# HKUST-Aerial-Robotics/FUEL

Measured on NVIDIA H100. Metric: replans_per_sec, higher is better.
Workload: dtype f64 (cost/gradient), i32+f32 (ESDF), u8 (frontier)

## Files before the change

fuel_b200/csrc/api.cu:

```cuda
#include "common.cuh"

#include <vector>

#include <math.h>
#include <stddef.h>
#include <new>

thread_local char g_fuelgpu_err[512] = "";

namespace {

__global__ void ingest_logodds_kernel(const int8_t* __restrict__ inflate, const double* __restrict__ lo,
                                      uint8_t* __restrict__ occ, int64_t n, double unknown_thr,
                                      double occ_thr) {
  const int64_t i = (int64_t)blockIdx.x * blockDim.x + threadIdx.x;
  if (i >= n) return;
  const double v = lo[i];
  int t = FUELGPU_FREE;
  if (v < unknown_thr)
    t = FUELGPU_UNKNOWN;
  else if (v > occ_thr)
    t = FUELGPU_OCCUPIED;
  occ[i] = (uint8_t)(t | ((inflate[i] == 1) ? 4 : 0));
}
// ... 558 lines not shown
  if (rc) return rc;
  rc = esdf_sample_impl(m, n, d_pos, d_d, d_g);
  if (rc) return rc;
  return st.download();
}

int fuelgpu_frontier_search(FuelMap* m, const double upd_min[3], const double upd_max[3],
                            const FuelFrontierParams* params, int32_t* n_clusters, int32_t* n_cells,
                            int32_t* n_filtered) {
  if (!m || !upd_min || !upd_max || !params || !n_clusters || !n_cells || !n_filtered)
    return fuel_fail(m, FUELGPU_EINVAL, "null argument");
  if (params->down_sample < 1) return fuel_fail(m, FUELGPU_EINVAL, "down_sample must be >= 1");
  FUEL_CUDA(m, cudaSetDevice(m->dev));
  cudaStream_t fs = frontier_stream(m);
  tbegin(m, T_FRONTIER, fs);
  int rc = frontier_search_impl(m, upd_min, upd_max, params, n_clusters, n_cells, n_filtered);
  tend(m, T_FRONTIER, fs);
  return rc;
}

int fuelgpu_frontier_search_begin(FuelMap* m, const double upd_min[3], const double upd_max[3],
                                  const FuelFrontierParams* params) {
  if (!m || !upd_min || !upd_max || !params) return fuel_fail(m, FUELGPU_EINVAL, "null argument");
  if (params->down_sample < 1) return fuel_fail(m, FUELGPU_EINVAL, "down_sample must be >= 1");
  FUEL_CUDA(m, cudaSetDevice(m->dev));
  cudaStream_t fs = frontier_stream(m);
  tbegin(m, T_FRONTIER, fs);
  return frontier_search_begin_impl(m, upd_min, upd_max, params);
}

int fuelgpu_frontier_search_end(FuelMap* m, int32_t* n_clusters, int32_t* n_cells, int32_t* n_filtered) {
  if (!m || !n_clusters || !n_cells || !n_filtered) return fuel_fail(m, FUELGPU_EINVAL, "null argument");
  FUEL_CUDA(m, cudaSetDevice(m->dev));
  int rc = frontier_search_end_impl(m, n_clusters, n_cells, n_filtered);
  tend(m, T_FRONTIER, frontier_stream_raw(m));
  return rc;
}

int fuelgpu_frontier_fetch(FuelMap* m, int32_t* cell_offsets, int32_t* cell_addr, int32_t* filt_offsets,
                           double* filtered, double* average, double* box_min, double* box_max) {
  if (!m) return fuel_fail(nullptr, FUELGPU_EINVAL, "null map");
  return frontier_fetch_impl(m, cell_offsets, cell_addr, filt_offsets, filtered, average, box_min, box_max);
}

int fuelgpu_frontier_candidates(FuelMap* m, const double upd_min[3], const double upd_max[3], const FuelFrontierParams* p,
                                int32_t z_lo, int32_t z_hi, int32_t* n_candidates) {
  if (!m || !upd_min || !upd_max || !p || !n_candidates) return fuel_fail(m, FUELGPU_EINVAL, "null argument");
  if (z_lo < 0 || z_hi >= m->g.nz || z_lo > z_hi) return fuel_fail(m, FUELGPU_EINVAL, "bad z range");
  FUEL_CUDA(m, cudaSetDevice(m->dev));
  tbegin(m, T_FRONTIER, frontier_stream(m));
  const int rc = frontier_candidates_impl(m, upd_min, upd_max, p, z_lo, z_hi, n_candidates);
  tend(m, T_FRONTIER, frontier_stream_raw(m));
  return rc;
}

int fuelgpu_frontier_candidates_fetch(FuelMap* m, int32_t n, int32_t* addr, uint8_t* cls) {
  if (!m || (n > 0 && (!addr || !cls))) return fuel_fail(m, FUELGPU_EINVAL, "null argument");
  FUEL_CUDA(m, cudaSetDevice(m->dev));
  return frontier_candidates_fetch_impl(m, n, addr, cls);
}

int fuelgpu_frontier_search_from_candidates(FuelMap* m, const double upd_min[3], const double upd_max[3],
                                            const FuelFrontierParams* p, int32_t n, const int32_t* addr, const uint8_t* cls,
                                            int32_t* n_clusters, int32_t* n_cells, int32_t* n_filtered) {
  if (!m || !upd_min || !upd_max || !p || !n_clusters || !n_cells || !n_filtered || (n > 0 && (!addr || !cls)))
    return fuel_fail(m, FUELGPU_EINVAL, "null argument");
  FUEL_CUDA(m, cudaSetDevice(m->dev));
  return frontier_search_from_candidates_impl(m, upd_min, upd_max, p, n, addr, cls, n_clusters, n_cells, n_filtered);
// ... 615 lines not shown
```

fuel_b200/csrc/common.cuh:

```cuda
#pragma once

#include <cuda_runtime.h>
#include <stdint.h>
#include <stdio.h>
#include <string.h>

#include <vector>

#include "fuelgpu.h"

#define FUELGPU_EDT_INF_I 0x3fffffff

struct Geom {
  int nx, ny, nz;
  double res, res_inv;
  double origin[3];
  double map_max[3];
  int box_min[3];
  int box_max[3];
  double box_mind[3], box_maxd[3];
};

enum { T_ESDF = 0, T_FRONTIER = 1, T_BSPLINE = 2, T_UPLOAD = 3, T_DOWNLOAD = 4, T_CHECK = 5, T_PARAM = 6, T_POLY = 7, T_COUNT = 8 };

struct FrontierState;
struct FusionState;
struct FuelMap;

template <typename T, bool Pinned = false>
struct DevBuf {
  T* p = nullptr;
  size_t cap = 0;
  int ensure(FuelMap* m, size_t n, bool* grew = nullptr);
  void release() {
    if (p) Pinned ? cudaFreeHost(p) : cudaFree(p);
    p = nullptr;
    cap = 0;
  }
};

// ... 4 lines not shown
  int sm_count;
  int64_t nvox;
  uint8_t* occ;
  float* dist;
  float* dist_neg;
  int8_t* flag;
  void* esdf_rec;
  void* esdf_p[2];
  size_t esdf_p_bytes;
  cudaStream_t esdf_aux;
  cudaEvent_t esdf_ev[2];
  DevBuf<uint8_t> stage;
  cudaStream_t own_stream, stream;
  cudaStream_t copy_stream;
  cudaEvent_t copy_ev;
  bool dist_ev_ok;
  cudaStream_t in_stream;
  cudaEvent_t in_ev;
  cudaEvent_t ev0[T_COUNT], ev1[T_COUNT];
  bool ev_valid[T_COUNT];
  FrontierState* fs;
  FusionState* fus;
  DevBuf<uint8_t> bs_buf;
  DevBuf<uint8_t, true> bs_pin;
  DevBuf<double> bs_grad;
  DevBuf<uint8_t> fr_scr;
  int bs_pend_B, bs_pend_nvar;
  size_t bs_pend_off;
  long long launches;
  char err[512];
  DevBuf<uint8_t> tc_buf;
  DevBuf<uint8_t> as_buf;
  size_t as_stride, as_warps;
};

extern thread_local char g_fuelgpu_err[512];

static inline int fuel_fail(FuelMap* m, int code, const char* fmt, const char* a = "", long long b = 0) {
  char* dst = m ? m->err : g_fuelgpu_err;
  snprintf(dst, 512, fmt, a, b);
  return code;
}

#define FUEL_CUDA(m, expr)                                                                     \
  do {                                                                                         \
    cudaError_t _e = (expr);                                                                   \
    if (_e != cudaSuccess) {                                                                   \
      char* _dst = (m) ? ((FuelMap*)(m))->err : g_fuelgpu_err;                                 \
      snprintf(_dst, 512, "CUDA error %s at %s:%d: %s", cudaGetErrorName(_e), __FILE__,        \
               __LINE__, cudaGetErrorString(_e));                                              \
      return _e == cudaErrorMemoryAllocation ? FUELGPU_ENOMEM : FUELGPU_ECUDA;                 \
    }                                                                                          \
  } while (0)

template <typename T, bool Pinned>
int DevBuf<T, Pinned>::ensure(FuelMap* m, size_t n, bool* grew) {
  if (grew) *grew = false;
  if (n <= cap) return 0;
  if (p) {
    FUEL_CUDA(m, cudaDeviceSynchronize());
    release();
  }
  const size_t want = n + n / 4 + 1024;
  T* q = nullptr;
  FUEL_CUDA(m, Pinned ? cudaMallocHost((void**)&q, want * sizeof(T)) : cudaMalloc((void**)&q, want * sizeof(T)));
  p = q;
  cap = want;
  if (grew) *grew = true;
  return 0;
}

static inline void tbegin(FuelMap* m, int t, cudaStream_t s = nullptr) { cudaEventRecord(m->ev0[t], s ? s : m->stream); }
static inline void tend(FuelMap* m, int t, cudaStream_t s = nullptr) {
  cudaEventRecord(m->ev1[t], s ? s : m->stream);
  m->ev_valid[t] = true;
}
#define FUEL_LAUNCHES(m, n) __atomic_fetch_add(&(m)->launches, (long long)(n), __ATOMIC_RELAXED)

__host__ __device__ static inline int64_t addr_of(const Geom& g, int x, int y, int z) {
  return ((int64_t)x * g.ny + y) * g.nz + z;
}

int esdf_update_impl(FuelMap* m, const int bmin[3], const int bmax[3], int flags);
void esdf_tile_scratch_sizes(int nx, int ny, int nz, size_t* rec_bytes, size_t* p_bytes, int* wc);
int esdf_tile_transform(FuelMap* m, const int lo[3], const int hi[3], int mode, float* out);
int edt_stage_zpack(cudaStream_t st, const uint8_t* occ, void* rec, int nxl, int ny, int nzc, int G, int64_t chunk_stride,
                    int mode);
int edt_stage_zy(cudaStream_t st, const void* rec, int nxl, int ny, int NW, int w0, int wn, int32_t* P, int64_t out_o,
                 int64_t out_bx, int64_t out_q);
int edt_stage_zy_scatter(cudaStream_t st, const void* rec, int nxl, int ny, int NW, int32_t* const* tab, int ntab, int wl,
                         int64_t out_o, int64_t out_bx, int64_t out_q);
int edt_stage_x(cudaStream_t st, const int32_t* P, int64_t in_o, int64_t in_bx, int64_t piece_stride, int piece_rows, int nx,
                int ny, int wn, float* out, int64_t out_o, int64_t out_bx, int64_t out_q, int lanes_total, float res,
                int discard);
int map_inflate_impl(FuelMap* m, const int bmin[3], const int bmax[3], int step, int ceil_id);
int esdf_sample_impl(FuelMap* m, int64_t n, const double* pos_dev, double* dist_dev, double* grad_dev);

int fusion_input_impl(FuelMap* m, const float* pts_host, int stride, int n, const double cam[3], const FuelFusionParams* p,
                      int32_t lbmin[3], int32_t lbmax[3]);
int fusion_input_depth_impl(FuelMap* m, const uint16_t* img_host, int rows, int cols, const FuelCameraParams* cp,
                            const double R[9], const double cam[3], const FuelFusionParams* p, int32_t lbmin[3],
                            int32_t lbmax[3], int32_t* proj_cnt);
int fusion_set_logodds(FuelMap* m, const double* logodds_host, double p_min, double p_occ);
int fusion_get_logodds(FuelMap* m, double* out);
void fusion_get_updated_box(FuelMap* m, double bmin[3], double bmax[3], int reset);
void fusion_state_destroy(FuelMap* m);
double* fusion_logodds_ptr(FuelMap* m, double* clamp_max_log);
void frontier_order_writer(FuelMap* m);
int frontier_set_cell_order(FuelMap* m, int order);
int frontier_candidates_impl(FuelMap* m, const double umin[3], const double umax[3], const FuelFrontierParams* p, int z_lo,
// ... 100 lines not shown
```

fuel_b200/csrc/frontier.cu:

```cuda
#include "common.cuh"

#include <cooperative_groups.h>

#include <algorithm>
#include <vector>

namespace cg = cooperative_groups;

namespace {

constexpr int NONE = 0x7fffffff;

struct FParams {
  int dom_lo[3], dom_n[3];
  int s_lo[3], s_hi[3];
  int z_min_idx;
  int cluster_min;
  double size_xy;
  float leaf, leaf_inv;
};

__device__ __forceinline__ int tri_at(const Geom& g, const uint8_t* __restrict__ occ, int x, int y,
                                      int z) {
  if (x < 0 || y < 0 || z < 0 || x >= g.nx || y >= g.ny || z >= g.nz) return -1;
// ... 1085 lines not shown
    *ctl.n_new = made;
  }
}

__global__ void relabel_kernel(Geom g, const int* __restrict__ k_addr, int* __restrict__ k_cl,
                               const ClusterMeta* __restrict__ meta, LevelCtl ctl) {
  if (*ctl.n_new == 0) return;
  relabel_item(g, k_addr, k_cl, meta, *ctl.K, *ctl.ccur, blockIdx.x * blockDim.x + threadIdx.x);
}

__global__ void next_level_kernel(ClusterMeta* meta, ClusterStat* st, LevelCtl ctl) {
  if (*ctl.n_new == 0) return;
  const int c = blockIdx.x * blockDim.x + threadIdx.x;
  clear_do_split_item(meta, *ctl.ccur, c);
  stat_reset_item(st, meta, *ctl.cnext, c);
}

__global__ void init_meta_kernel(ClusterMeta* meta, ClusterStat* st, LevelCtl ctl) {
  const int R = *ctl.R;
  const int c = blockIdx.x * blockDim.x + threadIdx.x;
  init_meta_item(meta, R, c);
  stat_reset_item(st, meta, R, c);
  if (c == 0) {
    *ctl.ccur = R;
    *ctl.c_final = R;
    *ctl.n_new = (R > 0 && *ctl.K > 0) ? 1 : 0;
  }
}


constexpr int SMALL_CTAS = 8;
constexpr int SMALL_CAP = 32768;
constexpr int SMALL_CCAP = 8192;
constexpr int RES_K0 = 12288, RES_C0 = 256;


__device__ __forceinline__ void mark_chunk_item(const int* __restrict__ seed, const int* __restrict__ csize, int cluster_min,
                                                int* __restrict__ root_mask, int* __restrict__ kept_mask, int n, int i) {
  bool kept = false, root = false;
  if (i < n) {
    const int s = seed[i];
    kept = s != NONE && csize[s] > cluster_min;
    root = kept && s == i;
  }
  const unsigned mk = __ballot_sync(0xffffffffu, kept), mr = __ballot_sync(0xffffffffu, root);
  if ((i & 31) == 0 && i < n) {
    kept_mask[i >> 5] = (int)mk;
    root_mask[i >> 5] = (int)mr;
  }
}
__device__ void chunk_scan_small(const int* __restrict__ root_mask, const int* __restrict__ kept_mask,
                                 int* __restrict__ root_off, int* __restrict__ kept_off, int nchunk,
                                 int* __restrict__ tot_root, int* __restrict__ tot_kept) {
  __shared__ unsigned wtot2[32];
  const int t = threadIdx.x, lane = t & 31, w = t >> 5;
  const unsigned v = t < nchunk ? ((unsigned)__popc((unsigned)root_mask[t]) << 16) + (unsigned)__popc((unsigned)kept_mask[t]) : 0u;
  unsigned inc = v;
#pragma unroll
  for (int o = 1; o < 32; o <<= 1) {
    const unsigned u = __shfl_up_sync(0xffffffffu, inc, o);
    if (lane >= o) inc += u;
  }
  if (lane == 31) wtot2[w] = inc;
  __syncthreads();
  if (w == 0) {
    const unsigned x = wtot2[lane];
    unsigned xi = x;
// ... 12 lines not shown
  if (t < nchunk) {
    const unsigned ex = wtot2[w] + inc - v;
    root_off[t] = (int)(ex >> 16);
    kept_off[t] = (int)(ex & 0xffffu);
  }
}
__device__ __forceinline__ void gather_chunk_item(const int* __restrict__ cell_addr, const int* __restrict__ seed,
                                                  const int* __restrict__ kept_mask, const int* __restrict__ kept_off,
                                                  const int* __restrict__ root_mask, const int* __restrict__ root_off,
                                                  int* __restrict__ k_addr, int* __restrict__ k_cl,
                                                  int* __restrict__ cellidx, int n, int i) {
  if (i >= n) return;
  const unsigned mk = (unsigned)kept_mask[i >> 5];
  const int a = cell_addr[i];
  if ((mk >> (i & 31)) & 1u) {
    const int k = kept_off[i >> 5] + __popc(mk & ((1u << (i & 31)) - 1u));
    const int s = seed[i];
    k_addr[k] = a;
    k_cl[k] = root_off[s >> 5] + __popc((unsigned)root_mask[s >> 5] & ((1u << (s & 31)) - 1u));
    cellidx[a] = k;
  } else {
    cellidx[a] = -1;
  }
}

struct SmallBufs {
  int *cell_addr, *parent, *claim, *csize, *seed, *is_root, *is_kept, *root_rank, *kept_off;
  uint8_t* cell_cls;
  int *k_addr, *k_cl, *k_leaf;
  float* k_cent;
  ClusterMeta* meta;
  ClusterStat* stat;
  int* counters;
  int* r_counters;
  ClusterMeta* r_meta;
  ClusterStat* r_stat;
  int *r_addr, *r_cl, *r_leaf;
  float* r_cent;
  int r_K, r_C;
};

__global__ void __cluster_dims__(SMALL_CTAS, 1, 1) __launch_bounds__(1024) cluster_small_kernel(Geom g, FParams fp, int8_t* __restrict__ flag,
                                                             int* __restrict__ cellidx, SmallBufs b) {
  cg::cluster_group cluster = cg::this_cluster();
  const int rank = (int)cluster.block_rank();
  const int tid = (((int)threadIdx.x >> 5) * SMALL_CTAS + rank) * 32 + ((int)threadIdx.x & 31);
  constexpr int NT = 1024 * SMALL_CTAS;
  const int n = b.counters[0];
#ifdef FUEL_PROF
  long long* prof = (long long*)(b.counters + 8);
  int pi = 0;
#define STAMP() do { if (tid == 0) { long long t_; asm volatile("mov.u64 %0, %%globaltimer;" : "=l"(t_)); prof[pi++] = t_; } } while (0)
#else
#define STAMP() do {} while (0)
#endif
  STAMP();
  if (n > SMALL_CAP) {
    if (tid == 0) {
      b.counters[4] = 1;
      b.r_counters[0] = n;
      b.r_counters[4] = 1;
    }
    return;
  }
#define FOR_ITEMS(i, N) for (int i = tid; i - tid < (N); i += NT)
  FOR_ITEMS(i, n) init_parent_item(b.parent, b.claim, b.csize, n, i);
  cluster.sync();
  STAMP();
  FOR_ITEMS(i, n) union_item(g, b.cell_addr, b.cell_cls, cellidx, b.parent, n, i);
  cluster.sync();
  STAMP();
  FOR_ITEMS(i, n) flatten_item(b.parent, b.cell_cls, n, i);
  cluster.sync();
  STAMP();
  FOR_ITEMS(i, n) claim_item(g, fp, b.cell_addr, b.cell_cls, cellidx, b.parent, b.claim, n, i);
  cluster.sync();
  STAMP();
  FOR_ITEMS(i, n) assign_item(b.cell_addr, b.cell_cls, b.parent, b.claim, b.seed, b.csize, flag, n, i);
  cluster.sync();
  STAMP();
  FOR_ITEMS(i, n) mark_chunk_item(b.seed, b.csize, fp.cluster_min, b.is_root, b.is_kept, n, i);
  cluster.sync();
  STAMP();
  if (rank == 0) chunk_scan_small(b.is_root, b.is_kept, b.root_rank, b.kept_off, (n + 31) >> 5, b.counters + 1, b.counters + 2);
  cluster.sync();
  STAMP();
  const int R = b.counters[1], K = b.counters[2];
  int C = R;
  int status = 0;
  if (R > 0 && K > 0) {
    FOR_ITEMS(i, n) gather_chunk_item(b.cell_addr, b.seed, b.is_kept, b.kept_off, b.is_root, b.root_rank, b.k_addr, b.k_cl,
                                      cellidx, n, i);
    FOR_ITEMS(c, R) {
      init_meta_item(b.meta, R, c);
      stat_reset_item(b.stat, b.meta, R, c);
    }
    cluster.sync();
    STAMP();
    for (int level = 0; level < 40; ++level) {
      if (2 * C > SMALL_CCAP) {
        status = 2;
        break;
      }
      FOR_ITEMS(k, K) stat_accum_item(g, b.k_addr, b.k_cl, b.meta, b.stat, K, k);
      cluster.sync();
      STAMP();
      FOR_ITEMS(c, C) mean_item(g, b.meta, b.stat, C, c);
      FOR_ITEMS(k, K) downsample_item<true>(g, fp, b.k_addr, b.k_cl, cellidx, b.meta, b.stat, b.k_cent, b.k_leaf, K, k);
      cluster.sync();
      STAMP();
      FOR_ITEMS(k, K) cov_item(g, b.k_cl, b.k_leaf, b.k_cent, b.meta, b.stat, K, k);
      cluster.sync();
      STAMP();
      FOR_ITEMS(c, C) pca_item(b.meta, b.stat, C, c);
      cluster.sync();
      STAMP();
      FOR_ITEMS(k, K) side_count_item(g, b.k_addr, b.k_cl, b.meta, b.stat, K, k);
      cluster.sync();
      STAMP();
      if (rank == 0) split_alloc(b.meta, b.stat, C, b.counters + 3);
      cluster.sync();
      STAMP();
      FOR_ITEMS(k, K) relabel_item(g, b.k_addr, b.k_cl, b.meta, K, C, k);
      cluster.sync();
      STAMP();
      const int n_new = b.counters[3];
      if (n_new == 0) break;
      FOR_ITEMS(c, C) clear_do_split_item(b.meta, C, c);
      C += n_new;
      FOR_ITEMS(c, C) stat_reset_item(b.stat, b.meta, C, c);
      cluster.sync();
      STAMP();
    }
  }
  FOR_ITEMS(i, n) reset_cellidx_item(b.cell_addr, cellidx, n, i);
  if (status == 0 && R > 0 && K > 0) {
    const int kp = min(K, b.r_K), cp = min(C, b.r_C);
    FOR_ITEMS(k, kp) {
      if (k < kp) {
        b.r_addr[k] = b.k_addr[k];
        b.r_cl[k] = b.k_cl[k];
        b.r_leaf[k] = b.k_leaf[k];
        b.r_cent[3 * k] = b.k_cent[3 * k];
        b.r_cent[3 * k + 1] = b.k_cent[3 * k + 1];
        b.r_cent[3 * k + 2] = b.k_cent[3 * k + 2];
      }
    }
    FOR_ITEMS(c, cp) {
      if (c < cp) {
        b.r_meta[c] = b.meta[c];
        b.r_stat[c] = b.stat[c];
      }
    }
  }
  if (tid == 0) {
    b.counters[4] = status;
    b.counters[5] = C;
    const int out[8] = { n, R, K, b.counters[3], status, C, b.counters[6], b.counters[7] };
#pragma unroll
    for (int j = 0; j < 8; ++j) b.r_counters[j] = out[j];
  }
#undef FOR_ITEMS
}

__global__ void is_changed_kernel(Geom g, const uint8_t* __restrict__ occ, const int* __restrict__ offs,
                                  const int* __restrict__ addr, uint8_t* __restrict__ changed, int* __restrict__ counts,
                                  int m) {
  const int c = blockIdx.x;
  if (c >= m) return;
  __shared__ int cnt;
  if (threadIdx.x == 0) cnt = 0;
  __syncthreads();
  int mine = 0;
  for (int i = offs[c] + threadIdx.x; i < offs[c + 1]; i += blockDim.x) {
    int x, y, z;
    addr_to_idx(g, addr[i], x, y, z);
    if (!frontier_pred(g, occ, x, y, z)) ++mine;
  }
  if (mine) atomicAdd(&cnt, mine);
  __syncthreads();
  if (threadIdx.x == 0) {
    if (changed) changed[c] = (uint8_t)(cnt > 0);
    if (counts) counts[c] = cnt;
  }
}

}

struct SweepPlan {
  bool words = false;
  unsigned nb = 0;
  size_t nmask = 0;
  int64_t ndom = 0;
  WordGeom wg;
};

struct HostView {
  const int *addr, *cl, *leaf;
  const float* cent;
  const ClusterMeta* meta;
  const ClusterStat* stat;
};

struct FrontierState {
  int* cellidx = nullptr;
  DevBuf<uint32_t> maskE, maskS;
  DevBuf<int> blockcnt, blockoff, scan_tot, scan_off;
  DevBuf<int> cell_addr, parent, claim, csize, seed, is_root, is_kept, root_rank, kept_off;
  DevBuf<uint8_t> cell_cls;
  DevBuf<int> k_addr, k_cl, k_leaf;
  DevBuf<float> k_cent;
  DevBuf<ClusterStat> stat;
  DevBuf<ClusterMeta> meta;
  DevBuf<char> res;
  bool small_ready = false;
  bool pend_active = false, pend_empty = true;
  FParams pend_fp;
  SweepPlan pend_plan;
  HostView pend_hv;
  cudaStream_t stream = nullptr;
  cudaEvent_t ev_in = nullptr;
  cudaEvent_t ev_out = nullptr;
  bool ev_out_valid = false;
  DevBuf<char, true> h_pin;
  int* d_counters = nullptr;
  std::vector<int32_t> h_cell_off, h_cell_addr, h_filt_off;
  std::vector<double> h_filtered, h_avg, h_bmin, h_bmax;
  int cell_order = FUELGPU_CELLS_BY_ADDRESS;
  float last_leaf = 0.f;
};

cudaStream_t frontier_stream_raw(FuelMap* m) { return m->fs->stream; }
cudaStream_t frontier_stream(FuelMap* m) {
  FrontierState* f = m->fs;
  cudaEventRecord(f->ev_in, m->stream);
  cudaStreamWaitEvent(f->stream, f->ev_in, 0);
  return f->stream;
}

int frontier_set_cell_order(FuelMap* m, int order) {
  if (order != FUELGPU_CELLS_BY_ADDRESS && order != FUELGPU_CELLS_BFS)
    return fuel_fail(m, FUELGPU_EINVAL, "unknown cell order");
  m->fs->cell_order = order;
  return 0;
}

void frontier_order_writer(FuelMap* m) {
  FrontierState* f = m->fs;
  if (f && f->ev_out_valid) cudaStreamWaitEvent(m->stream, f->ev_out, 0);
}

int frontier_state_create(FuelMap* m) {
  m->fs = new FrontierState();
  FUEL_CUDA(m, cudaStreamCreateWithFlags(&m->fs->stream, cudaStreamNonBlocking));
  FUEL_CUDA(m, cudaEventCreateWithFlags(&m->fs->ev_in, cudaEventDisableTiming));
  FUEL_CUDA(m, cudaEventCreateWithFlags(&m->fs->ev_out, cudaEventDisableTiming));
  FUEL_CUDA(m, cudaMalloc(&m->fs->cellidx, sizeof(int) * m->nvox));
  FUEL_CUDA(m, cudaMemsetAsync(m->fs->cellidx, 0xff, sizeof(int) * m->nvox, m->stream));
  FUEL_CUDA(m, cudaMalloc(&m->fs->d_counters, sizeof(int) * 8 + sizeof(long long) * 256));
  FUEL_CUDA(m, cudaMemsetAsync(m->fs->d_counters, 0, sizeof(int) * 8 + sizeof(long long) * 256, m->stream));
  return 0;
}

void frontier_state_destroy(FuelMap* m) {
  if (!m->fs) return;
  FrontierState* f = m->fs;
  if (f->stream) {
    cudaStreamSynchronize(f->stream);
    cudaStreamDestroy(f->stream);
  }
  if (f->ev_in) cudaEventDestroy(f->ev_in);
  if (f->ev_out) cudaEventDestroy(f->ev_out);
  if (f->cellidx) cudaFree(f->cellidx);
  if (f->d_counters) cudaFree(f->d_counters);
  f->h_pin.release();
  f->maskE.release(); f->maskS.release(); f->blockcnt.release(); f->blockoff.release();
  f->scan_tot.release(); f->scan_off.release();
  f->cell_addr.release(); f->parent.release(); f->claim.release(); f->csize.release();
  f->seed.release(); f->is_root.release(); f->is_kept.release(); f->root_rank.release();
  f->kept_off.release(); f->cell_cls.release(); f->k_addr.release(); f->k_cl.release();
  f->k_leaf.release(); f->k_cent.release(); f->stat.release(); f->meta.release(); f->res.release();
  delete f;
  m->fs = nullptr;
}

#define ENSURE(buf, n)                      \
  do {                                      \
    const int _rc = (buf).ensure(m, (n));   \
    if (_rc) return _rc;                    \
  } while (0)

static inline unsigned nblk(int64_t n, int b) { return (unsigned)((n + b - 1) / b); }

static int scan_ints(FuelMap* m, const int* in, int* out, int n, int* total) {
  FrontierState* f = m->fs;
  cudaStream_t s = m->fs->stream;
  if (n <= 4096) {
    scan_kernel<<<1, 1024, 0, s>>>(in, out, n, total);
    FUEL_LAUNCHES(m, 1);
    return 0;
  }
  const int nchunk = (n + 1023) / 1024;
  ENSURE(f->scan_tot, nchunk);
  ENSURE(f->scan_off, nchunk);
  scan_chunks_kernel<<<nchunk, 1024, 0, s>>>(in, out, n, f->scan_tot.p);
  scan_kernel<<<1, 1024, 0, s>>>(f->scan_tot.p, f->scan_off.p, nchunk, total);
  scan_add_kernel<<<nchunk, 1024, 0, s>>>(out, n, f->scan_off.p);
  FUEL_LAUNCHES(m, 3);
  return 0;
}

static SweepPlan sweep_plan(const Geom& g, const FParams& fp) {
  SweepPlan pl;
  pl.ndom = (int64_t)fp.dom_n[0] * fp.dom_n[1] * fp.dom_n[2];
// ... 316 lines not shown
    fp.s_hi[k] = ihi > nmax[k] - 1 ? nmax[k] - 1 : ihi;
    int dlo = g.box_min[k] < fp.s_lo[k] ? g.box_min[k] : fp.s_lo[k];
    int dhi = g.box_max[k] > fp.s_hi[k] ? g.box_max[k] : fp.s_hi[k];
    dlo = dlo < 0 ? 0 : dlo;
    dhi = dhi > nmax[k] - 1 ? nmax[k] - 1 : dhi;
    fp.dom_lo[k] = dlo;
    fp.dom_n[k] = dhi - dlo + 1;
    if (fp.dom_n[k] <= 0) {
      fp.dom_n[k] = 0;
    }
  }
  {
    int zi = 0;
    while (zi < g.nz && ((zi + 0.5) * g.res + g.origin[2]) < p->min_z) ++zi;
    fp.z_min_idx = zi;
  }
  fp.cluster_min = p->cluster_min;
  fp.size_xy = p->cluster_size_xy;
  fp.leaf = (float)(g.res * p->down_sample);
  f->last_leaf = fp.leaf;
  fp.leaf_inv = 1.0f / fp.leaf;
  f->pend_fp = fp;
  *out = fp;
}

static void frontier_clear_results(FrontierState* f) {
  f->h_cell_off.assign(1, 0);
  f->h_cell_addr.clear();
  f->h_filt_off.assign(1, 0);
  f->h_filtered.clear();
  f->h_avg.clear();
  f->h_bmin.clear();
  f->h_bmax.clear();
  f->pend_active = false;
  f->pend_empty = true;
}

int frontier_search_begin_impl(FuelMap* m, const double umin[3], const double umax[3],
                               const FuelFrontierParams* p) {
  FrontierState* f = m->fs;
  const Geom& g = m->g;
  cudaStream_t s = m->fs->stream;
  FParams fp;
  frontier_make_params(m, umin, umax, p, &fp);

  f->h_cell_off.assign(1, 0);
  f->h_cell_addr.clear();
  f->h_filt_off.assign(1, 0);
  f->h_filtered.clear();
  f->h_avg.clear();
  f->h_bmin.clear();
  f->h_bmax.clear();
  f->pend_active = false;
  f->pend_empty = true;

  const SweepPlan pl = sweep_plan(g, fp);
  if (pl.ndom <= 0) return 0;
  f->pend_empty = false;
  {
    const int rc = sweep_classify(m, fp, pl, s);
    if (rc) return rc;
  }
  {
    ENSURE(f->cell_addr, SMALL_CAP); ENSURE(f->cell_cls, SMALL_CAP); ENSURE(f->parent, SMALL_CAP);
    ENSURE(f->claim, SMALL_CAP); ENSURE(f->csize, SMALL_CAP); ENSURE(f->seed, SMALL_CAP);
    ENSURE(f->is_root, SMALL_CAP); ENSURE(f->is_kept, SMALL_CAP); ENSURE(f->root_rank, SMALL_CAP);
    ENSURE(f->kept_off, SMALL_CAP); ENSURE(f->k_addr, SMALL_CAP); ENSURE(f->k_cl, SMALL_CAP);
    ENSURE(f->k_leaf, SMALL_CAP); ENSURE(f->k_cent, (size_t)3 * SMALL_CAP);
    ENSURE(f->meta, SMALL_CCAP); ENSURE(f->stat, SMALL_CCAP);
    const ResultLayout rl = result_layout(RES_K0, RES_C0);
    ENSURE(f->res, 64 + rl.bytes);
    sweep_compact(m, fp, pl, f->cellidx, SMALL_CAP, s);
    SmallBufs sb;
    sb.cell_addr = f->cell_addr.p; sb.parent = f->parent.p; sb.claim = f->claim.p; sb.csize = f->csize.p;
    sb.seed = f->seed.p; sb.is_root = f->is_root.p; sb.is_kept = f->is_kept.p; sb.root_rank = f->root_rank.p;
    sb.kept_off = f->kept_off.p; sb.cell_cls = f->cell_cls.p; sb.k_addr = f->k_addr.p; sb.k_cl = f->k_cl.p;
    sb.k_leaf = f->k_leaf.p; sb.k_cent = f->k_cent.p; sb.meta = f->meta.p; sb.stat = f->stat.p;
    sb.counters = f->d_counters;
    {
      char* rb = f->res.p + 64;
      sb.r_counters = (int*)f->res.p;
      sb.r_meta = (ClusterMeta*)(rb + rl.meta); sb.r_stat = (ClusterStat*)(rb + rl.stat);
      sb.r_addr = (int*)(rb + rl.addr); sb.r_cl = (int*)(rb + rl.cl); sb.r_leaf = (int*)(rb + rl.leaf);
      sb.r_cent = (float*)(rb + rl.cent);
      sb.r_K = RES_K0;
      sb.r_C = RES_C0;
    }
    cluster_small_kernel<<<SMALL_CTAS, 1024, 0, s>>>(g, fp, m->flag, f->cellidx, sb);
    FUEL_LAUNCHES(m, 1);
    ENSURE(f->h_pin, 64 + rl.bytes);
    FUEL_CUDA(m, cudaMemcpyAsync(f->h_pin.p, f->res.p, 64 + rl.bytes, cudaMemcpyDeviceToHost, s));
    result_view(rl, f->h_pin.p + 64, &f->pend_hv);
    f->pend_fp = fp;
    f->pend_plan = pl;
    f->pend_active = true;
  }
  cudaEventRecord(f->ev_out, f->stream);
  f->ev_out_valid = true;
  return 0;
}

int frontier_search_end_impl(FuelMap* m, int32_t* n_clusters, int32_t* n_cells, int32_t* n_filtered) {
  FrontierState* f = m->fs;
  const Geom& g = m->g;
  cudaStream_t s = m->fs->stream;
  *n_clusters = *n_cells = *n_filtered = 0;
  if (f->pend_empty || !f->pend_active) {
    f->pend_active = false;
    return 0;
  }
  f->pend_active = false;
  const FParams fp = f->pend_fp;
  const SweepPlan pl = f->pend_plan;
  int n_cand = 0;
  {
    const int* cnt = (const int*)f->h_pin.p;
    HostView& hv = f->pend_hv;
    FUEL_CUDA(m, cudaStreamSynchronize(s));
    n_cand = cnt[0];
    if (n_cand == 0) return 0;
    if (cnt[4] == 0) {
      const int R = cnt[1], K = cnt[2], C = cnt[5];
      if (R == 0 || K == 0) return 0;
      if (K <= RES_K0 && C <= RES_C0) return frontier_build_csr(m, K, C, hv, n_clusters, n_cells, n_filtered);
      return frontier_marshal(m, K, C, n_clusters, n_cells, n_filtered);
    }
    if (cnt[4] == 1) {
      reset_cellidx_kernel<<<nblk(SMALL_CAP, 256), 256, 0, s>>>(f->cell_addr.p, f->cellidx, SMALL_CAP);
      FUEL_LAUNCHES(m, 1);
    }
  }

  ENSURE(f->cell_addr, n_cand); ENSURE(f->cell_cls, n_cand); ENSURE(f->parent, n_cand);
  ENSURE(f->claim, n_cand); ENSURE(f->csize, n_cand); ENSURE(f->seed, n_cand);
  ENSURE(f->is_root, n_cand); ENSURE(f->is_kept, n_cand); ENSURE(f->root_rank, n_cand);
  ENSURE(f->kept_off, n_cand);

  sweep_compact(m, fp, pl, f->cellidx, n_cand, s);
  return frontier_cluster_large(m, fp, n_cand, n_clusters, n_cells, n_filtered);
}

static int frontier_cluster_large(FuelMap* m, const FParams& fp, int n_cand, int32_t* n_clusters, int32_t* n_cells,
                                  int32_t* n_filtered) {
  FrontierState* f = m->fs;
  const Geom& g = m->g;
  cudaStream_t s = m->fs->stream;
  ENSURE(f->parent, n_cand);
  ENSURE(f->claim, n_cand); ENSURE(f->csize, n_cand); ENSURE(f->seed, n_cand);
  ENSURE(f->is_root, n_cand); ENSURE(f->is_kept, n_cand); ENSURE(f->root_rank, n_cand);
  ENSURE(f->kept_off, n_cand);
  ENSURE(f->k_addr, n_cand); ENSURE(f->k_cl, n_cand); ENSURE(f->k_leaf, n_cand); ENSURE(f->k_cent, (size_t)3 * n_cand);
  ENSURE(f->meta, (size_t)n_cand + 1024);
  ENSURE(f->stat, (size_t)n_cand + 1024);
  const unsigned cb = nblk(n_cand, 256);
  init_parent_kernel<<<cb, 256, 0, s>>>(f->parent.p, f->claim.p, f->csize.p, n_cand);
  union_kernel<<<cb, 256, 0, s>>>(g, f->cell_addr.p, f->cell_cls.p, f->cellidx, f->parent.p, n_cand);
  flatten_kernel<<<cb, 256, 0, s>>>(f->parent.p, f->cell_cls.p, n_cand);
// ... 79 lines not shown
    if (rc) return rc;
  }
  int n = 0;
  FUEL_CUDA(m, cudaMemcpyAsync(&n, f->d_counters, sizeof(int), cudaMemcpyDeviceToHost, s));
  FUEL_CUDA(m, cudaStreamSynchronize(s));
  if (n > 0) {
    ENSURE(f->cell_addr, n);
    ENSURE(f->cell_cls, n);
    sweep_compact(m, fp, pl, nullptr, n, s);
    FUEL_CUDA(m, cudaGetLastError());
  }
  *n_out = n;
  return 0;
}

int frontier_candidates_fetch_impl(FuelMap* m, int32_t n, int32_t* addr, uint8_t* cls) {
  FrontierState* f = m->fs;
  if (n <= 0) return 0;
  cudaStream_t s = f->stream;
  FUEL_CUDA(m, cudaMemcpyAsync(addr, f->cell_addr.p, sizeof(int) * n, cudaMemcpyDeviceToHost, s));
  FUEL_CUDA(m, cudaMemcpyAsync(cls, f->cell_cls.p, n, cudaMemcpyDeviceToHost, s));
  FUEL_CUDA(m, cudaStreamSynchronize(s));
  return 0;
}

int frontier_search_from_candidates_impl(FuelMap* m, const double umin[3], const double umax[3], const FuelFrontierParams* p,
                                         int32_t n, const int32_t* addr, const uint8_t* cls, int32_t* n_clusters,
                                         int32_t* n_cells, int32_t* n_filtered) {
  FrontierState* f = m->fs;
  cudaStream_t s = frontier_stream(m);
  FParams fp;
  frontier_make_params(m, umin, umax, p, &fp);
  frontier_clear_results(f);
  *n_clusters = *n_cells = *n_filtered = 0;
  if (n <= 0) return 0;
  for (int i = 1; i < n; ++i)
    if (addr[i] <= addr[i - 1]) return fuel_fail(m, FUELGPU_EINVAL, "candidate addresses must be strictly ascending");
  if (addr[0] < 0 || (int64_t)addr[n - 1] >= m->nvox) return fuel_fail(m, FUELGPU_EINVAL, "candidate address outside the map");
  ENSURE(f->cell_addr, n);
  ENSURE(f->cell_cls, n);
  FUEL_CUDA(m, cudaMemcpyAsync(f->cell_addr.p, addr, sizeof(int) * n, cudaMemcpyHostToDevice, s));
  FUEL_CUDA(m, cudaMemcpyAsync(f->cell_cls.p, cls, n, cudaMemcpyHostToDevice, s));
  set_cellidx_kernel<<<nblk(n, 256), 256, 0, s>>>(f->cell_addr.p, f->cellidx, n);
  FUEL_LAUNCHES(m, 1);
  FUEL_CUDA(m, cudaMemcpyAsync(f->d_counters, &n, sizeof(int), cudaMemcpyHostToDevice, s));
  const int rc = frontier_cluster_large(m, fp, n, n_clusters, n_cells, n_filtered);
  cudaEventRecord(f->ev_out, f->stream);
  f->ev_out_valid = true;
  return rc;
}

int frontier_search_impl(FuelMap* m, const double umin[3], const double umax[3],
                         const FuelFrontierParams* p, int32_t* n_clusters, int32_t* n_cells,
                         int32_t* n_filtered) {
  int rc = frontier_search_begin_impl(m, umin, umax, p);
  if (rc) return rc;
  return frontier_search_end_impl(m, n_clusters, n_cells, n_filtered);
}

int frontier_fetch_impl(FuelMap* m, int32_t* cell_offsets, int32_t* cell_addr, int32_t* filt_offsets,
                        double* filtered, double* average, double* box_min, double* box_max) {
  FrontierState* f = m->fs;
  if (cell_offsets) memcpy(cell_offsets, f->h_cell_off.data(), sizeof(int32_t) * f->h_cell_off.size());
  if (cell_addr) memcpy(cell_addr, f->h_cell_addr.data(), sizeof(int32_t) * f->h_cell_addr.size());
  if (filt_offsets) memcpy(filt_offsets, f->h_filt_off.data(), sizeof(int32_t) * f->h_filt_off.size());
  if (filtered) memcpy(filtered, f->h_filtered.data(), sizeof(double) * f->h_filtered.size());
  if (average) memcpy(average, f->h_avg.data(), sizeof(double) * f->h_avg.size());
  if (box_min) memcpy(box_min, f->h_bmin.data(), sizeof(double) * f->h_bmin.size());
  if (box_max) memcpy(box_max, f->h_bmax.data(), sizeof(double) * f->h_bmax.size());
  return 0;
}

int frontier_is_changed_impl(FuelMap* m, int32_t mcl, const int32_t* offs, const int32_t* addr,
                             uint8_t* changed, int32_t* counts) {
  if (mcl <= 0) return 0;
  const int ncell = offs[mcl];
  const size_t nci = (size_t)(ncell > 0 ? ncell : 1);
  int rc = m->fr_scr.ensure(m, sizeof(int) * ((size_t)2 * mcl + 1 + nci) + mcl + 16);
  if (rc) return rc;
  int* d_off = (int*)m->fr_scr.p;
  int* d_addr = d_off + mcl + 1;
  int* d_cnt = d_addr + nci;
  uint8_t* d_ch = (uint8_t*)(d_cnt + mcl);
  cudaStream_t s = m->fs->stream;
  FUEL_CUDA(m, cudaMemcpyAsync(d_off, offs, sizeof(int) * (mcl + 1), cudaMemcpyHostToDevice, s));
  if (ncell > 0) FUEL_CUDA(m, cudaMemcpyAsync(d_addr, addr, sizeof(int) * ncell, cudaMemcpyHostToDevice, s));
  is_changed_kernel<<<mcl, 128, 0, s>>>(m->g, m->occ, d_off, d_addr, d_ch, d_cnt, mcl);
  FUEL_LAUNCHES(m, 1);
  if (changed) FUEL_CUDA(m, cudaMemcpyAsync(changed, d_ch, mcl, cudaMemcpyDeviceToHost, s));
  if (counts) FUEL_CUDA(m, cudaMemcpyAsync(counts, d_cnt, sizeof(int) * mcl, cudaMemcpyDeviceToHost, s));
  FUEL_CUDA(m, cudaStreamSynchronize(s));
  return 0;
}

#ifdef FUEL_PROF
extern "C" __attribute__((visibility("default"))) int fuelgpu_debug_frontier_prof(FuelMap* m, long long* out,
                                                                                  int n) {
  cudaMemcpy(out, (long long*)(m->fs->d_counters + 8), sizeof(long long) * n, cudaMemcpyDeviceToHost);
  return 0;
}
#endif
```

Measured before the change: 2093.

## Assemble frontier CSR results on device in the small cluster kernel

```diff
diff --git a/fuel_b200/csrc/api.cu b/fuel_b200/csrc/api.cu
--- a/fuel_b200/csrc/api.cu
+++ b/fuel_b200/csrc/api.cu
@@ -614,8 +614,18 @@
 int fuelgpu_frontier_search_end(FuelMap* m, int32_t* n_clusters, int32_t* n_cells, int32_t* n_filtered) {
   if (!m || !n_clusters || !n_cells || !n_filtered) return fuel_fail(m, FUELGPU_EINVAL, "null argument");
   FUEL_CUDA(m, cudaSetDevice(m->dev));
+#ifdef FUEL_PROF
+  const double t0 = prof_now_us();
+#endif
   int rc = frontier_search_end_impl(m, n_clusters, n_cells, n_filtered);
+#ifdef FUEL_PROF
+  const double t1 = prof_now_us();
+  m->end_prof_us[1] = t1 - t0 - m->end_prof_us[0];
+#endif
   tend(m, T_FRONTIER, frontier_stream_raw(m));
+#ifdef FUEL_PROF
+  m->end_prof_us[2] = prof_now_us() - t1;
+#endif
   return rc;
 }
 
diff --git a/fuel_b200/csrc/common.cuh b/fuel_b200/csrc/common.cuh
--- a/fuel_b200/csrc/common.cuh
+++ b/fuel_b200/csrc/common.cuh
@@ -6,6 +6,9 @@
 #include <string.h>
 
 #include <vector>
+#ifdef FUEL_PROF
+#include <chrono>
+#endif
 
 #include "fuelgpu.h"
 
@@ -76,6 +79,9 @@
   DevBuf<uint8_t> tc_buf;
   DevBuf<uint8_t> as_buf;
   size_t as_stride, as_warps;
+#ifdef FUEL_PROF
+  double end_prof_us[3];
+#endif
 };
 
 extern thread_local char g_fuelgpu_err[512];
@@ -120,6 +126,12 @@
   m->ev_valid[t] = true;
 }
 #define FUEL_LAUNCHES(m, n) __atomic_fetch_add(&(m)->launches, (long long)(n), __ATOMIC_RELAXED)
+#ifdef FUEL_PROF
+static inline double prof_now_us() {
+  return 1e-3 * (double)std::chrono::duration_cast<std::chrono::nanoseconds>(
+                    std::chrono::steady_clock::now().time_since_epoch()).count();
+}
+#endif
 
 __host__ __device__ static inline int64_t addr_of(const Geom& g, int x, int y, int z) {
   return ((int64_t)x * g.ny + y) * g.nz + z;
diff --git a/fuel_b200/csrc/frontier.cu b/fuel_b200/csrc/frontier.cu
--- a/fuel_b200/csrc/frontier.cu
+++ b/fuel_b200/csrc/frontier.cu
@@ -1141,7 +1141,19 @@
 constexpr int SMALL_CTAS = 8;
 constexpr int SMALL_CAP = 32768;
 constexpr int SMALL_CCAP = 8192;
-constexpr int RES_K0 = 12288, RES_C0 = 256;
+constexpr int RES_K0 = 12288, RES_C0 = 256, RES_F0 = 4096;
+constexpr size_t al16(size_t b) { return (b + 15) & ~(size_t)15; }
+constexpr size_t RB_CELL_OFF = 64;
+constexpr size_t RB_FILT_OFF = RB_CELL_OFF + al16(sizeof(int) * (RES_C0 + 1));
+constexpr size_t RB_AVG = RB_FILT_OFF + al16(sizeof(int) * (RES_C0 + 1));
+constexpr size_t RB_BOX = RB_AVG + al16(sizeof(double) * 3 * RES_C0);
+constexpr size_t RB_ADDR = RB_BOX + al16(sizeof(int) * 6 * RES_C0);
+constexpr size_t RB_FILT = RB_ADDR + al16(sizeof(int) * RES_K0);
+constexpr size_t RB_BYTES = RB_FILT + al16(sizeof(double) * 3 * RES_F0);
+constexpr size_t ASM_SCR = 3 * RES_C0 + 2 * RES_K0 + 3 * RES_F0;
+constexpr unsigned TAG_PAD = 0x8000u;
+static_assert(RES_C0 <= 256 && RES_C0 <= SMALL_CTAS * 32, "cluster ids fit a tag byte, one warp per cluster");
+static_assert(RES_K0 % 128 == 0 && sizeof(int) * RES_F0 <= sizeof(unsigned short) * RES_K0, "tail's shared memory");
 
 
 __device__ __forceinline__ void mark_chunk_item(const int* __restrict__ seed, const int* __restrict__ csize, int cluster_min,
@@ -1220,13 +1232,136 @@
   ClusterMeta* meta;
   ClusterStat* stat;
   int* counters;
-  int* r_counters;
-  ClusterMeta* r_meta;
-  ClusterStat* r_stat;
-  int *r_addr, *r_cl, *r_leaf;
-  float* r_cent;
-  int r_K, r_C;
+  char* res;
+  int* scr;
+  int assemble;
 };
+
+__device__ __forceinline__ void tail_count_item(const int* __restrict__ k_cl, const int* __restrict__ k_leaf,
+                                                int* __restrict__ cnt_cell, int* __restrict__ cnt_filt, int K, int k) {
+  const int c = k < K ? k_cl[k] : -1;
+  const int cf = (k < K && k_leaf[k] >= 0) ? c : -1;
+  const unsigned pc = __match_any_sync(0xffffffffu, c), pf = __match_any_sync(0xffffffffu, cf);
+  const int lane = k & 31;
+  if (c >= 0 && lane == __ffs(pc) - 1) atomicAdd(cnt_cell + c, __popc(pc));
+  if (cf >= 0 && lane == __ffs(pf) - 1) atomicAdd(cnt_filt + cf, __popc(pf));
+}
+__device__ __forceinline__ void tail_rank_warp(const ClusterMeta* __restrict__ meta, int* __restrict__ crank, int C, int c,
+                                               int lane) {
+  const int r0 = meta[c].root;
+  const unsigned p0 = meta[c].path;
+  int lt = 0;
+  for (int c2 = lane; c2 < C; c2 += 32) {
+    const int r2 = meta[c2].root;
+    const unsigned p2 = meta[c2].path;
+    lt += r2 < r0 || (r2 == r0 && (p2 < p0 || (p2 == p0 && c2 < c)));
+  }
+  lt = __reduce_add_sync(0xffffffffu, lt);
+  if (lane == 0) crank[c] = lt;
+}
+__device__ __forceinline__ void tail_tags(const int* __restrict__ k_cl, const int* __restrict__ k_leaf,
+                                          unsigned short* __restrict__ tag, int K) {
+  const int Kp = (K + 127) & ~127;
+  for (int k = threadIdx.x; k < Kp; k += blockDim.x)
+    tag[k] = (unsigned short)(k < K ? (unsigned)k_cl[k] | (k_leaf[k] >= 0 ? 0x100u : 0u) : TAG_PAD);
+}
+__device__ __forceinline__ void tail_place_warp(const ClusterMeta* __restrict__ meta, const ClusterStat* __restrict__ st,
+                                                const unsigned short* __restrict__ tag, int* __restrict__ scr,
+                                                char* __restrict__ res, int K, int C, int c, int lane) {
+  const int *cnt_cell = scr, *cnt_filt = scr + RES_C0, *crank = scr + 2 * RES_C0;
+  int* pos = scr + 3 * RES_C0;
+  int* fpos = pos + RES_K0;
+  const int r = crank[c];
+  int co = 0, fo = 0;
+  for (int c2 = lane; c2 < C; c2 += 32) {
+    if (crank[c2] < r) {
+      co += cnt_cell[c2];
+      fo += cnt_filt[c2];
+    }
+  }
+  co = __reduce_add_sync(0xffffffffu, co);
+  fo = __reduce_add_sync(0xffffffffu, fo);
+  int* cell_off = (int*)(res + RB_CELL_OFF);
+  int* filt_off = (int*)(res + RB_FILT_OFF);
+  if (lane == 0) {
+    cell_off[r] = co;
+    filt_off[r] = fo;
+    if (r == C - 1) {
+      cell_off[C] = co + cnt_cell[c];
+      filt_off[C] = fo + cnt_filt[c];
+    }
+  }
+  if (lane < 3) {
+    ((double*)(res + RB_AVG))[3 * r + lane] = meta[c].mean[lane];
+    ((int*)(res + RB_BOX))[6 * r + lane] = st[c].lo[lane];
+    ((int*)(res + RB_BOX))[6 * r + 3 + lane] = st[c].hi[lane];
+  }
+  const int Kp = (K + 127) & ~127;
+  for (int base = 0; base < Kp; base += 128) {
+    const uint2 w = *(const uint2*)(tag + base + 4 * lane);
+    const unsigned t[4] = { w.x & 0xffffu, w.x >> 16, w.y & 0xffffu, w.y >> 16 };
+    unsigned mine = 0, filt = 0;
+#pragma unroll
+    for (int j = 0; j < 4; ++j) {
+      if ((t[j] & 0x80ffu) == (unsigned)c) {
+        mine |= 1u << j;
+        if (t[j] & 0x100u) filt |= 1u << j;
+      }
+    }
+    if (!__any_sync(0xffffffffu, mine)) continue;
+    const unsigned v = (unsigned)__popc(mine) | ((unsigned)__popc(filt) << 16);
+    unsigned inc = v;
+#pragma unroll
+    for (int o = 1; o < 32; o <<= 1) {
+      const unsigned u = __shfl_up_sync(0xffffffffu, inc, o);
+      if (lane >= o) inc += u;
+    }
+    const unsigned tot = __shfl_sync(0xffffffffu, inc, 31), ex = inc - v;
+    int pm = co + (int)(ex & 0xffffu), pf = fo + (int)(ex >> 16);
+#pragma unroll
+    for (int j = 0; j < 4; ++j) {
+      if ((mine >> j) & 1u) {
+        pos[base + 4 * lane + j] = pm++;
+        if ((filt >> j) & 1u) fpos[base + 4 * lane + j] = pf++;
+      }
+    }
+    co += (int)(tot & 0xffffu);
+    fo += (int)(tot >> 16);
+  }
+}
+__device__ __forceinline__ void tail_scatter_item(const int* __restrict__ k_addr, const int* __restrict__ k_cl,
+                                                  const int* __restrict__ k_leaf, const int* __restrict__ scr,
+                                                  int* __restrict__ f_k, int* __restrict__ f_leaf, int* __restrict__ f_r,
+                                                  char* __restrict__ res, int K, int k) {
+  if (k >= K) return;
+  const int *crank = scr + 2 * RES_C0, *pos = scr + 3 * RES_C0, *fpos = pos + RES_K0;
+  ((int*)(res + RB_ADDR))[pos[k]] = k_addr[k];
+  const int lf = k_leaf[k];
+  if (lf >= 0) {
+    const int s = fpos[k];
+    f_k[s] = k;
+    f_leaf[s] = lf;
+    f_r[s] = crank[k_cl[k]];
+  }
+}
+__device__ __forceinline__ void tail_filtered_item(const float* __restrict__ k_cent, const int* __restrict__ f_k,
+                                                   const int* __restrict__ s_leaf, const int* __restrict__ f_r,
+                                                   char* __restrict__ res, int NF, int i) {
+  if (i >= NF) return;
+  const int* filt_off = (const int*)(res + RB_FILT_OFF);
+  const int r = f_r[i], lo = filt_off[r], hi = filt_off[r + 1], lf = s_leaf[i];
+  int pos = lo;
+#pragma unroll 4
+  for (int j = lo; j < hi; ++j) {
+    const int l2 = s_leaf[j];
+    pos += l2 < lf || (l2 == lf && j < i);
+  }
+  const int k = f_k[i];
+  double* out = (double*)(res + RB_FILT);
+  out[3 * pos] = (double)k_cent[3 * k];
+  out[3 * pos + 1] = (double)k_cent[3 * k + 1];
+  out[3 * pos + 2] = (double)k_cent[3 * k + 2];
+}
 
 __global__ void __cluster_dims__(SMALL_CTAS, 1, 1) __launch_bounds__(1024) cluster_small_kernel(Geom g, FParams fp, int8_t* __restrict__ flag,
                                                              int* __restrict__ cellidx, SmallBufs b) {
@@ -1243,11 +1378,12 @@
 #define STAMP() do {} while (0)
 #endif
   STAMP();
+  int* r_counters = (int*)b.res;
   if (n > SMALL_CAP) {
     if (tid == 0) {
       b.counters[4] = 1;
-      b.r_counters[0] = n;
-      b.r_counters[4] = 1;
+      r_counters[0] = n;
+      r_counters[4] = 1;
     }
     return;
   }
@@ -1283,6 +1419,7 @@
       init_meta_item(b.meta, R, c);
       stat_reset_item(b.stat, b.meta, R, c);
     }
+    if (b.assemble) FOR_ITEMS(c, 2 * RES_C0) if (c < 2 * RES_C0) b.scr[c] = 0;
     cluster.sync();
     STAMP();
     for (int level = 0; level < 40; ++level) {
@@ -1322,31 +1459,41 @@
     }
   }
   FOR_ITEMS(i, n) reset_cellidx_item(b.cell_addr, cellidx, n, i);
-  if (status == 0 && R > 0 && K > 0) {
-    const int kp = min(K, b.r_K), cp = min(C, b.r_C);
-    FOR_ITEMS(k, kp) {
-      if (k < kp) {
-        b.r_addr[k] = b.k_addr[k];
-        b.r_cl[k] = b.k_cl[k];
-        b.r_leaf[k] = b.k_leaf[k];
-        b.r_cent[3 * k] = b.k_cent[3 * k];
-        b.r_cent[3 * k + 1] = b.k_cent[3 * k + 1];
-        b.r_cent[3 * k + 2] = b.k_cent[3 * k + 2];
-      }
-    }
-    FOR_ITEMS(c, cp) {
-      if (c < cp) {
-        b.r_meta[c] = b.meta[c];
-        b.r_stat[c] = b.stat[c];
-      }
+  int assembled = 0, NF = 0;
+  if (b.assemble && status == 0 && R > 0 && K > 0 && K <= RES_K0 && C <= RES_C0) {
+    __shared__ __align__(16) unsigned short s_tag[RES_K0];
+    int* f_k = b.scr + 3 * RES_C0 + 2 * RES_K0;
+    int* f_leaf = f_k + RES_F0;
+    int* f_r = f_leaf + RES_F0;
+    const int gw = tid >> 5, lane = tid & 31;
+    FOR_ITEMS(k, K) tail_count_item(b.k_cl, b.k_leaf, b.scr, b.scr + RES_C0, K, k);
+    if (gw < C) tail_rank_warp(b.meta, b.scr + 2 * RES_C0, C, gw, lane);
+    cluster.sync();
+    STAMP();
+    tail_tags(b.k_cl, b.k_leaf, s_tag, K);
+    __syncthreads();
+    if (gw < C) tail_place_warp(b.meta, b.stat, s_tag, b.scr, b.res, K, C, gw, lane);
+    cluster.sync();
+    STAMP();
+    NF = ((const int*)(b.res + RB_FILT_OFF))[C];
+    if (NF <= RES_F0) {
+      FOR_ITEMS(k, K) tail_scatter_item(b.k_addr, b.k_cl, b.k_leaf, b.scr, f_k, f_leaf, f_r, b.res, K, k);
+      cluster.sync();
+      STAMP();
+      int* s_leaf = (int*)s_tag;
+      for (int i = threadIdx.x; i < NF; i += blockDim.x) s_leaf[i] = f_leaf[i];
+      __syncthreads();
+      FOR_ITEMS(i, NF) tail_filtered_item(b.k_cent, f_k, s_leaf, f_r, b.res, NF, i);
+      STAMP();
+      assembled = 1;
     }
   }
   if (tid == 0) {
     b.counters[4] = status;
     b.counters[5] = C;
-    const int out[8] = { n, R, K, b.counters[3], status, C, b.counters[6], b.counters[7] };
-#pragma unroll
-    for (int j = 0; j < 8; ++j) b.r_counters[j] = out[j];
+    const int out[10] = { n, R, K, b.counters[3], status, C, b.counters[6], b.counters[7], assembled, NF };
+#pragma unroll
+    for (int j = 0; j < 10; ++j) r_counters[j] = out[j];
   }
 #undef FOR_ITEMS
 }
@@ -1401,16 +1548,18 @@
   DevBuf<ClusterStat> stat;
   DevBuf<ClusterMeta> meta;
   DevBuf<char> res;
-  bool small_ready = false;
+  DevBuf<int> asm_scr;
   bool pend_active = false, pend_empty = true;
   FParams pend_fp;
   SweepPlan pend_plan;
-  HostView pend_hv;
   cudaStream_t stream = nullptr;
   cudaEvent_t ev_in = nullptr;
   cudaEvent_t ev_out = nullptr;
   bool ev_out_valid = false;
   DevBuf<char, true> h_pin;
+  DevBuf<char, true> h_res[2];
+  int pend_blk = 0;
+  int res_blk = -1;
   int* d_counters = nullptr;
   std::vector<int32_t> h_cell_off, h_cell_addr, h_filt_off;
   std::vector<double> h_filtered, h_avg, h_bmin, h_bmax;
@@ -1468,6 +1617,7 @@
   f->seed.release(); f->is_root.release(); f->is_kept.release(); f->root_rank.release();
   f->kept_off.release(); f->cell_cls.release(); f->k_addr.release(); f->k_cl.release();
   f->k_leaf.release(); f->k_cent.release(); f->stat.release(); f->meta.release(); f->res.release();
+  f->asm_scr.release(); f->h_res[0].release(); f->h_res[1].release();
   delete f;
   m->fs = nullptr;
 }
@@ -1850,8 +2000,12 @@
   f->h_avg.clear();
   f->h_bmin.clear();
   f->h_bmax.clear();
-  f->pend_active = false;
-  f->pend_empty = true;
+  f->res_blk = -1;
+}
+
+static bool frontier_host_csr() {
+  const char* e = getenv("FUELGPU_FRONTIER_HOST_CSR");
+  return e && *e && strcmp(e, "0") != 0;
 }
 
 int frontier_search_begin_impl(FuelMap* m, const double umin[3], const double umax[3],
@@ -1862,13 +2016,6 @@
   FParams fp;
   frontier_make_params(m, umin, umax, p, &fp);
 
-  f->h_cell_off.assign(1, 0);
-  f->h_cell_addr.clear();
-  f->h_filt_off.assign(1, 0);
-  f->h_filtered.clear();
-  f->h_avg.clear();
-  f->h_bmin.clear();
-  f->h_bmax.clear();
   f->pend_active = false;
   f->pend_empty = true;
 
@@ -1886,8 +2033,10 @@
     ENSURE(f->kept_off, SMALL_CAP); ENSURE(f->k_addr, SMALL_CAP); ENSURE(f->k_cl, SMALL_CAP);
     ENSURE(f->k_leaf, SMALL_CAP); ENSURE(f->k_cent, (size_t)3 * SMALL_CAP);
     ENSURE(f->meta, SMALL_CCAP); ENSURE(f->stat, SMALL_CCAP);
-    const ResultLayout rl = result_layout(RES_K0, RES_C0);
-    ENSURE(f->res, 64 + rl.bytes);
+    ENSURE(f->res, RB_BYTES); ENSURE(f->asm_scr, ASM_SCR);
+    const bool assemble = !frontier_host_csr() && f->cell_order != FUELGPU_CELLS_BFS;
+    const int blk = f->res_blk == 0 ? 1 : 0;
+    ENSURE(f->h_res[blk], RB_BYTES);
     sweep_compact(m, fp, pl, f->cellidx, SMALL_CAP, s);
     SmallBufs sb;
     sb.cell_addr = f->cell_addr.p; sb.parent = f->parent.p; sb.claim = f->claim.p; sb.csize = f->csize.p;
@@ -1895,20 +2044,13 @@
     sb.kept_off = f->kept_off.p; sb.cell_cls = f->cell_cls.p; sb.k_addr = f->k_addr.p; sb.k_cl = f->k_cl.p;
     sb.k_leaf = f->k_leaf.p; sb.k_cent = f->k_cent.p; sb.meta = f->meta.p; sb.stat = f->stat.p;
     sb.counters = f->d_counters;
-    {
-      char* rb = f->res.p + 64;
-      sb.r_counters = (int*)f->res.p;
-      sb.r_meta = (ClusterMeta*)(rb + rl.meta); sb.r_stat = (ClusterStat*)(rb + rl.stat);
-      sb.r_addr = (int*)(rb + rl.addr); sb.r_cl = (int*)(rb + rl.cl); sb.r_leaf = (int*)(rb + rl.leaf);
-      sb.r_cent = (float*)(rb + rl.cent);
-      sb.r_K = RES_K0;
-      sb.r_C = RES_C0;
-    }
+    sb.res = f->res.p;
+    sb.scr = f->asm_scr.p;
+    sb.assemble = assemble ? 1 : 0;
     cluster_small_kernel<<<SMALL_CTAS, 1024, 0, s>>>(g, fp, m->flag, f->cellidx, sb);
     FUEL_LAUNCHES(m, 1);
-    ENSURE(f->h_pin, 64 + rl.bytes);
-    FUEL_CUDA(m, cudaMemcpyAsync(f->h_pin.p, f->res.p, 64 + rl.bytes, cudaMemcpyDeviceToHost, s));
-    result_view(rl, f->h_pin.p + 64, &f->pend_hv);
+    FUEL_CUDA(m, cudaMemcpyAsync(f->h_res[blk].p, f->res.p, assemble ? RB_BYTES : RB_CELL_OFF, cudaMemcpyDeviceToHost, s));
+    f->pend_blk = blk;
     f->pend_fp = fp;
     f->pend_plan = pl;
     f->pend_active = true;
@@ -1923,6 +2065,10 @@
   const Geom& g = m->g;
   cudaStream_t s = m->fs->stream;
   *n_clusters = *n_cells = *n_filtered = 0;
+  frontier_clear_results(f);
+#ifdef FUEL_PROF
+  m->end_prof_us[0] = 0.0;
+#endif
   if (f->pend_empty || !f->pend_active) {
     f->pend_active = false;
     return 0;
@@ -1932,15 +2078,26 @@
   const SweepPlan pl = f->pend_plan;
   int n_cand = 0;
   {
-    const int* cnt = (const int*)f->h_pin.p;
-    HostView& hv = f->pend_hv;
+    const int* cnt = (const int*)f->h_res[f->pend_blk].p;
+#ifdef FUEL_PROF
+    const double t0 = prof_now_us();
+#endif
     FUEL_CUDA(m, cudaStreamSynchronize(s));
+#ifdef FUEL_PROF
+    m->end_prof_us[0] = prof_now_us() - t0;
+#endif
     n_cand = cnt[0];
     if (n_cand == 0) return 0;
     if (cnt[4] == 0) {
       const int R = cnt[1], K = cnt[2], C = cnt[5];
       if (R == 0 || K == 0) return 0;
-      if (K <= RES_K0 && C <= RES_C0) return frontier_build_csr(m, K, C, hv, n_clusters, n_cells, n_filtered);
+      if (cnt[8]) {
+        *n_clusters = C;
+        *n_cells = K;
+        *n_filtered = cnt[9];
+        f->res_blk = f->pend_blk;
+        return 0;
+      }
       return frontier_marshal(m, K, C, n_clusters, n_cells, n_filtered);
     }
     if (cnt[4] == 1) {
@@ -2086,6 +2243,8 @@
   FParams fp;
   frontier_make_params(m, umin, umax, p, &fp);
   frontier_clear_results(f);
+  f->pend_active = false;
+  f->pend_empty = true;
   *n_clusters = *n_cells = *n_filtered = 0;
   if (n <= 0) return 0;
   for (int i = 1; i < n; ++i)
@@ -2115,6 +2274,24 @@
 int frontier_fetch_impl(FuelMap* m, int32_t* cell_offsets, int32_t* cell_addr, int32_t* filt_offsets,
                         double* filtered, double* average, double* box_min, double* box_max) {
   FrontierState* f = m->fs;
+  if (f->res_blk >= 0) {
+    const char* rb = f->h_res[f->res_blk].p;
+    const int* cnt = (const int*)rb;
+    const int K = cnt[2], C = cnt[5], NF = cnt[9];
+    const Geom& g = m->g;
+    if (cell_offsets) memcpy(cell_offsets, rb + RB_CELL_OFF, sizeof(int32_t) * (C + 1));
+    if (cell_addr) memcpy(cell_addr, rb + RB_ADDR, sizeof(int32_t) * K);
+    if (filt_offsets) memcpy(filt_offsets, rb + RB_FILT_OFF, sizeof(int32_t) * (C + 1));
+    if (filtered) memcpy(filtered, rb + RB_FILT, sizeof(double) * 3 * NF);
+    if (average) memcpy(average, rb + RB_AVG, sizeof(double) * 3 * C);
+    const int* box = (const int*)(rb + RB_BOX);
+    for (int r = 0; r < C; ++r)
+      for (int a = 0; a < 3; ++a) {
+        if (box_min) box_min[3 * r + a] = (box[6 * r + a] + 0.5) * g.res + g.origin[a];
+        if (box_max) box_max[3 * r + a] = (box[6 * r + 3 + a] + 0.5) * g.res + g.origin[a];
+      }
+    return 0;
+  }
   if (cell_offsets) memcpy(cell_offsets, f->h_cell_off.data(), sizeof(int32_t) * f->h_cell_off.size());
   if (cell_addr) memcpy(cell_addr, f->h_cell_addr.data(), sizeof(int32_t) * f->h_cell_addr.size());
   if (filt_offsets) memcpy(filt_offsets, f->h_filt_off.data(), sizeof(int32_t) * f->h_filt_off.size());
@@ -2153,4 +2330,8 @@
   cudaMemcpy(out, (long long*)(m->fs->d_counters + 8), sizeof(long long) * n, cudaMemcpyDeviceToHost);
   return 0;
 }
+extern "C" __attribute__((visibility("default"))) int fuelgpu_debug_frontier_end_prof(FuelMap* m, double* out) {
+  for (int i = 0; i < 3; ++i) out[i] = m->end_prof_us[i];
+  return 0;
+}
 #endif
```

Result: faster. 2503 (median of 6 runs) (+19.6%).
